# PaddlePaddle/PaddleFleetX

Measured on AMD Instinct MI355X. Metric: tokens/sec/GPU GPT-3-6.7B pretrain, DP2×TP2×PP2 at 1/2/4/8 MI355X, higher is better.
Workload: dtype bf16; 1 GPU; model=GPT-6.7B, global_batch=32, seq_len=1024, micro_batch=16, parallelism=dp1tp1pp1

## Files before the change

### csrc/attention.hip

```cpp
#include "common.h"

#include <torch/extension.h>
#include <ATen/hip/HIPContext.h>

namespace {

typedef __attribute__((ext_vector_type(8))) __bf16 bf8;
typedef __attribute__((ext_vector_type(4))) float f4;
typedef __attribute__((ext_vector_type(8))) short short8v;

#define MFMA_BF16(a, b, c) __builtin_amdgcn_mfma_f32_16x16x32_bf16(a, b, c, 0, 0, 0)

constexpr int TILE = 64;
constexpr int NWAVES = 4;
constexpr int BLOCKT = NWAVES * WAVE;
constexpr int PAD = 8;

constexpr int FW_WAVES = 8;
constexpr int FW_BLOCKT = FW_WAVES * WAVE;
constexpr int QTILE = FW_WAVES * 16;

struct Strided {
  const __hip_bfloat16* p;
  long bs, hs, rs;
  DEV_INLINE const __hip_bfloat16* at(int b, int h) const {
    return p + (long)b * bs + (long)h * hs;
  }
};
struct StridedMut {
  __hip_bfloat16* p;
  long bs, hs, rs;
  DEV_INLINE __hip_bfloat16* at(int b, int h) const {
    return p + (long)b * bs + (long)h * hs;
  }
};

template <int D>
DEV_INLINE void stage_rowmajor(const __hip_bfloat16* __restrict__ g, long rs,
                               int nvalid, unsigned short* lds) {
  constexpr int RS = D + PAD;
  constexpr int NV = TILE * D / 8;
  for (int v = threadIdx.x; v < NV; v += BLOCKT) {
    int row = v / (D / 8);
    int col = (v % (D / 8)) * 8;
    short4v lo = {0, 0, 0, 0}, hi = {0, 0, 0, 0};
    if (row < nvalid) {
      const unsigned short* src = (const unsigned short*)g + (long)row * rs + col;
      lo = *reinterpret_cast<const short4v*>(src);
      hi = *reinterpret_cast<const short4v*>(src + 4);
    }
    *reinterpret_cast<short4v*>(lds + row * RS + col) = lo;
    *reinterpret_cast<short4v*>(lds + row * RS + col + 4) = hi;
  }
}

template <int D>
DEV_INLINE void stage_both(const __hip_bfloat16* __restrict__ g, long rs,
                           int nvalid, unsigned short* lds_rm,
                           unsigned short* lds_tr) {
  constexpr int RSM = D + PAD;
  constexpr int RST = TILE + PAD;
  constexpr int NV = TILE * D / 8;
  for (int v = threadIdx.x; v < NV; v += BLOCKT) {
    int row = v / (D / 8);
    int col = (v % (D / 8)) * 8;
    short4v lo = {0, 0, 0, 0}, hi = {0, 0, 0, 0};
    if (row < nvalid) {
      const unsigned short* src = (const unsigned short*)g + (long)row * rs + col;
      lo = *reinterpret_cast<const short4v*>(src);
      hi = *reinterpret_cast<const short4v*>(src + 4);
    }
    *reinterpret_cast<short4v*>(lds_rm + row * RSM + col) = lo;
    *reinterpret_cast<short4v*>(lds_rm + row * RSM + col + 4) = hi;
    unsigned short tmp[8];
    *reinterpret_cast<short4v*>(tmp) = lo;
    *reinterpret_cast<short4v*>(tmp + 4) = hi;
#pragma unroll
    for (int j = 0; j < 8; ++j) lds_tr[(col + j) * RST + row] = tmp[j];
  }
}

template <int D>
DEV_INLINE void load_a_frags(const __hip_bfloat16* __restrict__ g, long rs,
                             int row0, int nvalid, int lane, bf8* frags) {
  int row = row0 + (lane & 15);
  int d0 = (lane >> 4) * 8;
#pragma unroll
  for (int kc = 0; kc < D / 32; ++kc) {
    bf8 f = {};
    if (row < nvalid) {
      const unsigned short* src =
          (const unsigned short*)g + (long)row * rs + kc * 32 + d0;
      union { short4v v[2]; bf8 b; } u;
      u.v[0] = *reinterpret_cast<const short4v*>(src);
      u.v[1] = *reinterpret_cast<const short4v*>(src + 4);
      f = u.b;
    }
    frags[kc] = f;
  }
}

DEV_INLINE bf8 read_b_frag(const unsigned short* lds, int row_stride, int col0,
                           int k0, int lane) {
  const unsigned short* p =
      lds + (col0 + (lane & 15)) * row_stride + k0 + (lane >> 4) * 8;
  union { short4v v[2]; bf8 b; } u;
  u.v[0] = *reinterpret_cast<const short4v*>(p);
  u.v[1] = *reinterpret_cast<const short4v*>(p + 4);
  return u.b;
}

DEV_INLINE bf8 read_a_frag_lds(const unsigned short* lds, int row_stride,
                               int k0, int lane) {
  const unsigned short* p =
      lds + (lane & 15) * row_stride + k0 + (lane >> 4) * 8;
  union { short4v v[2]; bf8 b; } u;
  u.v[0] = *reinterpret_cast<const short4v*>(p);
  u.v[1] = *reinterpret_cast<const short4v*>(p + 4);
  return u.b;
}

template <int D, bool CAUSAL, bool DROP>
__global__ __launch_bounds__(FW_BLOCKT) void attn_fwd_kernel(
    Strided q, Strided k, Strided v, StridedMut o, float* __restrict__ lse_out,
    int H, int S, float scale, int kv_total, int n_home,
    unsigned drop_thresh, float drop_inv_keep, unsigned seed0,
    unsigned seed1) {
  constexpr int KRS = D + PAD;
  constexpr int VRS = TILE + 4;
  constexpr int NDT = D / 16;
  constexpr int KSZ = TILE * KRS;
  constexpr int VSZ = D * VRS;

  __shared__ unsigned short smem[2 * KSZ + 2 * VSZ];
  unsigned short* k_lds = smem;
  unsigned short* vt_lds = smem + 2 * KSZ;

  const int b = blockIdx.x / H, hh = blockIdx.x % H;
  const long bh = blockIdx.x;
  const int wid = threadIdx.x / WAVE;
  const int lane = threadIdx.x % WAVE;

  const __hip_bfloat16* qp = q.at(b, hh);
  const __hip_bfloat16* kp = k.at(b, hh);
  const __hip_bfloat16* vp = v.at(b, hh);

  auto run_qtile = [&](const int qt) {

  constexpr int RB = 2;
  const int qrow0 = qt * (QTILE * RB) + wid * (16 * RB);
  bf8 qfrag[RB][D / 32];
#pragma unroll
  for (int rb = 0; rb < RB; ++rb)
    load_a_frags<D>(qp, q.rs, qrow0 + rb * 16, S, lane, qfrag[rb]);

  f4 oacc[RB][NDT];
#pragma unroll
  for (int rb = 0; rb < RB; ++rb)
#pragma unroll
    for (int i = 0; i < NDT; ++i) oacc[rb][i] = f4{0.f, 0.f, 0.f, 0.f};
  float m_r[RB][1], l_r[RB][1];
#pragma unroll
  for (int rb = 0; rb < RB; ++rb) { m_r[rb][0] = -INFINITY; l_r[rb][0] = 0.f; }

  const int ccol = lane & 15;
  const int crow4 = (lane >> 4) * 4;

  const int kv_tiles = CAUSAL
      ? min(kv_total, (qt * QTILE * RB + QTILE * RB - 1) / TILE + 1)
      : kv_total;

  constexpr int TPR = D / 16;
  const int st_row = threadIdx.x / TPR;
  const int st_col = (threadIdx.x % TPR) * 16;
  const bool st_on = st_row < TILE;
  constexpr int VCB = D / 4;
  const int vb_row = (threadIdx.x / VCB) * 4;
  const int vb_col = (threadIdx.x % VCB) * 4;
  const bool vb_on = vb_row < TILE;
  short8v kreg[2];
  short4v vblk[4];

  auto load_kv = [&](int kv0) {
#pragma unroll
    for (int h2 = 0; h2 < 2; ++h2) kreg[h2] = short8v{};
#pragma unroll
    for (int r = 0; r < 4; ++r) vblk[r] = short4v{};
    const int krow = kv0 + st_row;
    if (st_on && krow < S) {
      const unsigned short* ks = (const unsigned short*)kp +
                                 (long)krow * k.rs + st_col;
      kreg[0] = *reinterpret_cast<const short8v*>(ks);
      kreg[1] = *reinterpret_cast<const short8v*>(ks + 8);
    }
    if (vb_on) {
#pragma unroll
      for (int r = 0; r < 4; ++r) {
        const int vrow = kv0 + vb_row + r;
// ... 181 lines not shown
          oacc[rb][dt] = MFMA_BF16(pa[rb][kc], vb, oacc[rb][dt]);
      }
    }

    if (have_next)
      write_kv(k_lds + (cur ^ 1) * KSZ, vt_lds + (cur ^ 1) * VSZ);
    __syncthreads();
  }

  __hip_bfloat16* op = o.at(b, hh);
#pragma unroll
  for (int rb = 0; rb < RB; ++rb) {
    float inv_own = (l_r[rb][0] > 0.f) ? 1.f / l_r[rb][0] : 0.f;
    float inv4[4];
#pragma unroll
    for (int r = 0; r < 4; ++r) inv4[r] = __shfl(inv_own, crow4 + r, WAVE);
    if ((lane >> 4) == 0 && lse_out) {
      int qrow = qrow0 + rb * 16 + ccol;
      if (qrow < S)
        lse_out[bh * (long)S + qrow] =
            (l_r[rb][0] > 0.f) ? m_r[rb][0] + logf(l_r[rb][0]) : -INFINITY;
    }
#pragma unroll
    for (int r = 0; r < 4; ++r) {
      int qrow = qrow0 + rb * 16 + crow4 + r;
      if (qrow >= S) continue;
      unsigned short* orow = (unsigned short*)op + (long)qrow * o.rs;
#pragma unroll
      for (int dt = 0; dt < NDT; dt += 2) {
        unsigned int u = cvt_pk_bf16(oacc[rb][dt][r] * inv4[r],
                                     oacc[rb][dt + 1][r] * inv4[r]);
        orow[dt * 16 + ccol] = (unsigned short)u;
        orow[(dt + 1) * 16 + ccol] = (unsigned short)(u >> 16);
      }
    }
  }
  };

  const int n_home_abs = n_home < 0 ? -n_home : n_home;
  run_qtile(blockIdx.y);
  if (n_home < 0) {
    const int qt2 = (n_home_abs - 1) - (int)blockIdx.y;
    if (qt2 != (int)blockIdx.y && qt2 >= 0) {
      __syncthreads();
      run_qtile(qt2);
    }
  }
}

__global__ void attn_bwd_delta_kernel(Strided dout, Strided o,
                                      float* __restrict__ delta, long rows,
                                      int H, int S, int D) {
  constexpr int GROUPS = BLOCKT / 16;
  long row = (long)blockIdx.x * GROUPS + threadIdx.x / 16;
  if (row >= rows) return;
  int s = (int)(row % S);
  long bh = row / S;
  int hh = (int)(bh % H);
  int b = (int)(bh / H);
  int lane16 = threadIdx.x % 16;
  const unsigned short* dp =
      (const unsigned short*)dout.at(b, hh) + (long)s * dout.rs;
  const unsigned short* op = (const unsigned short*)o.at(b, hh) + (long)s * o.rs;
  float acc = 0.f;
  for (int i = lane16 * 4; i < D; i += 16 * 4) {
    short4v dv = *reinterpret_cast<const short4v*>(dp + i);
    short4v ov = *reinterpret_cast<const short4v*>(op + i);
#pragma unroll
    for (int j = 0; j < 4; ++j)
      acc += bf_raw2f(((unsigned short*)&dv)[j]) *
             bf_raw2f(((unsigned short*)&ov)[j]);
  }
  acc = group16_reduce_sum(acc);
  if (lane16 == 0) delta[bh * (long)S + s] = acc;
}

template <int D, bool CAUSAL, bool DROP>
__global__ __launch_bounds__(FW_BLOCKT) void attn_bwd_dkv_kernel(
    Strided q, Strided k, Strided v, Strided dout,
    const float* __restrict__ lse, const float* __restrict__ delta,
    StridedMut dk, StridedMut dv, int H, int S, float scale, int q_tiles,
    int n_home, unsigned drop_thresh, float drop_inv_keep, unsigned seed0,
    unsigned seed1) {
  constexpr int RS = D + PAD;
  constexpr int TS = TILE + PAD;
  constexpr int TRS = TILE + 4;
  constexpr int NDT = D / 16;
  constexpr int QSZ = TILE * RS;
  constexpr int TSZ = D * TRS;

  __shared__ unsigned short q_lds[2 * QSZ];
  __shared__ unsigned short qt_lds[2 * TSZ];
  __shared__ unsigned short do_lds[2 * QSZ];
  __shared__ unsigned short dot_lds[2 * TSZ];
  __shared__ unsigned short p_lds[FW_WAVES * 16 * TS];
  __shared__ float lsed_lds[2][2 * TILE];

  const int b = blockIdx.x / H, hh = blockIdx.x % H;
  const long bh = blockIdx.x;
  const int wid = threadIdx.x / WAVE;
  const int lane = threadIdx.x % WAVE;

  const __hip_bfloat16* qp = q.at(b, hh);
  const __hip_bfloat16* kp = k.at(b, hh);
  const __hip_bfloat16* vp = v.at(b, hh);
  const __hip_bfloat16* dop = dout.at(b, hh);

  auto run_kvtile = [&](const int kt) {
  const int kvrow0 = kt * QTILE + wid * 16;
  bf8 kfrag[D / 32], vfrag[D / 32];
  load_a_frags<D>(kp, k.rs, kvrow0, S, lane, kfrag);
  load_a_frags<D>(vp, v.rs, kvrow0, S, lane, vfrag);

  f4 dvacc[NDT], dkacc[NDT];
#pragma unroll
  for (int i = 0; i < NDT; ++i) {
    dvacc[i] = f4{0.f, 0.f, 0.f, 0.f};
    dkacc[i] = f4{0.f, 0.f, 0.f, 0.f};
  }

  const int ccol = lane & 15;
  const int crow4 = (lane >> 4) * 4;
  const int my_kvrow = kvrow0 + crow4;
  unsigned short* myp = p_lds + wid * 16 * TS;

  constexpr int TPR = D / 16;
  const int st_row = threadIdx.x / TPR;
  const int st_col = (threadIdx.x % TPR) * 16;
  const bool st_on = st_row < TILE;
  constexpr int VCB = D / 4;
  const int vb_row = (threadIdx.x / VCB) * 4;
  const int vb_col = (threadIdx.x % VCB) * 4;
  const bool vb_on = vb_row < TILE;
  short8v qreg[2], dreg[2];
  short4v qblk[4], dblk[4];
  float lse_s = 0.f, dlt_s = 0.f;

  const int qt_first = CAUSAL ? (kt * QTILE) / TILE : 0;

  auto issue_loads = [&](int q0) {
#pragma unroll
    for (int h2 = 0; h2 < 2; ++h2) { qreg[h2] = short8v{}; dreg[h2] = short8v{}; }
#pragma unroll
    for (int r = 0; r < 4; ++r) { qblk[r] = short4v{}; dblk[r] = short4v{}; }
    const int row = q0 + st_row;
    if (st_on && row < S) {
      const unsigned short* qs = (const unsigned short*)qp + (long)row * q.rs + st_col;
      const unsigned short* ds = (const unsigned short*)dop + (long)row * dout.rs + st_col;
      qreg[0] = *reinterpret_cast<const short8v*>(qs);
      qreg[1] = *reinterpret_cast<const short8v*>(qs + 8);
      dreg[0] = *reinterpret_cast<const short8v*>(ds);
      dreg[1] = *reinterpret_cast<const short8v*>(ds + 8);
    }
    if (vb_on) {
#pragma unroll
      for (int r = 0; r < 4; ++r) {
        const int vrow = q0 + vb_row + r;
        if (vrow < S) {
          qblk[r] = *reinterpret_cast<const short4v*>(
              (const unsigned short*)qp + (long)vrow * q.rs + vb_col);
          dblk[r] = *reinterpret_cast<const short4v*>(
              (const unsigned short*)dop + (long)vrow * dout.rs + vb_col);
        }
      }
    }
    const int li = threadIdx.x;
    if (li < TILE) {
      int qi = q0 + li;
      lse_s = (qi < S) ? lse[bh * (long)S + qi] : 0.f;
      dlt_s = (qi < S) ? delta[bh * (long)S + qi] : 0.f;
    }
  };
  auto write_tiles = [&](int buf) {
    unsigned short* qd = q_lds + buf * QSZ;
    unsigned short* dd = do_lds + buf * QSZ;
    unsigned short* qtd = qt_lds + buf * TSZ;
    unsigned short* dtd = dot_lds + buf * TSZ;
    if (st_on) {
      *reinterpret_cast<short8v*>(qd + st_row * RS + st_col) = qreg[0];
      *reinterpret_cast<short8v*>(qd + st_row * RS + st_col + 8) = qreg[1];
      *reinterpret_cast<short8v*>(dd + st_row * RS + st_col) = dreg[0];
      *reinterpret_cast<short8v*>(dd + st_row * RS + st_col + 8) = dreg[1];
    }
    if (vb_on) {
#pragma unroll
      for (int c = 0; c < 4; ++c) {
        short4v tq = {qblk[0][c], qblk[1][c], qblk[2][c], qblk[3][c]};
        short4v td = {dblk[0][c], dblk[1][c], dblk[2][c], dblk[3][c]};
        *reinterpret_cast<short4v*>(qtd + (vb_col + c) * TRS + vb_row) = tq;
        *reinterpret_cast<short4v*>(dtd + (vb_col + c) * TRS + vb_row) = td;
      }
    }
    if (threadIdx.x < TILE) {
      lsed_lds[buf][threadIdx.x] = lse_s;
      lsed_lds[buf][TILE + threadIdx.x] = dlt_s;
    }
  };

  issue_loads(qt_first * TILE);
  write_tiles(0);
  __syncthreads();

  for (int qt = qt_first; qt < q_tiles; ++qt) {
    const int q0 = qt * TILE;
    const int cur = (qt - qt_first) & 1;
    const unsigned short* qb_lds = q_lds + cur * QSZ;
    const unsigned short* db_lds = do_lds + cur * QSZ;
    const unsigned short* qtb_lds = qt_lds + cur * TSZ;
    const unsigned short* dtb_lds = dot_lds + cur * TSZ;
    const float* lsed_b = lsed_lds[cur];
    const bool have_next = (qt + 1) < q_tiles;
    if (have_next) issue_loads(q0 + TILE);

    const bool active = !CAUSAL || (q0 + TILE - 1 >= kvrow0);
    f4 pt[4], dpt[4];
    if (active) {
      unsigned dmask[4];
#pragma unroll
      for (int ct = 0; ct < 4; ++ct) {
        f4 acc = {0.f, 0.f, 0.f, 0.f};
#pragma unroll
        for (int kc = 0; kc < D / 32; ++kc) {
          bf8 qb = read_b_frag(qb_lds, RS, ct * 16, kc * 32, lane);
          acc = MFMA_BF16(kfrag[kc], qb, acc);
        }
        int qcol = q0 + ct * 16 + ccol;
        float l = lsed_b[ct * 16 + ccol];
#pragma unroll
        for (int r = 0; r < 4; ++r) {
          int kvr = my_kvrow + r;
          float p = 0.f;
          if ((!CAUSAL || qcol >= kvr) && qcol < S && kvr < S)
            p = __expf(acc[r] * scale - l);
          pt[ct][r] = p;
        }
        if constexpr (DROP) {
          philox4 r4 = philox4x32_10((unsigned)qcol,
                                     (unsigned)(my_kvrow >> 2),
                                     (unsigned)bh, seed1, seed0, seed1);
          const unsigned rr[4] = {r4.x, r4.y, r4.z, r4.w};
          unsigned m = 0;
#pragma unroll
          for (int r = 0; r < 4; ++r)
            if (rr[r] >= drop_thresh) m |= (1u << r);
          dmask[ct] = m;
        }
      }

#pragma unroll
      for (int ct = 0; ct < 4; ++ct)
#pragma unroll
        for (int r = 0; r < 4; r += 2) {
          float p0 = pt[ct][r], p1 = pt[ct][r + 1];
          if constexpr (DROP) {
            p0 = (dmask[ct] >> r) & 1 ? p0 * drop_inv_keep : 0.f;
            p1 = (dmask[ct] >> (r + 1)) & 1 ? p1 * drop_inv_keep : 0.f;
          }
          unsigned int u = cvt_pk_bf16(p0, p1);
          unsigned short* base = myp + (crow4 + r) * TS + ct * 16 + ccol;
          base[0] = (unsigned short)u;
          base[TS] = (unsigned short)(u >> 16);
        }
#pragma unroll
      for (int kc = 0; kc < 2; ++kc) {
        bf8 pa = read_a_frag_lds(myp, TS, kc * 32, lane);
#pragma unroll
        for (int dt = 0; dt < NDT; ++dt) {
          bf8 db = read_b_frag(dtb_lds, TRS, dt * 16, kc * 32, lane);
          dvacc[dt] = MFMA_BF16(pa, db, dvacc[dt]);
        }
      }

#pragma unroll
      for (int ct = 0; ct < 4; ++ct) {
        f4 acc = {0.f, 0.f, 0.f, 0.f};
#pragma unroll
        for (int kc = 0; kc < D / 32; ++kc) {
          bf8 db = read_b_frag(db_lds, RS, ct * 16, kc * 32, lane);
          acc = MFMA_BF16(vfrag[kc], db, acc);
        }
        dpt[ct] = acc;
      }

#pragma unroll
      for (int ct = 0; ct < 4; ++ct) {
        float dlt = lsed_b[TILE + ct * 16 + ccol];
        float ds[4];
#pragma unroll
        for (int r = 0; r < 4; ++r) {
          float dp = dpt[ct][r];
          if constexpr (DROP)
            dp = (dmask[ct] >> r) & 1 ? dp * drop_inv_keep : 0.f;
          ds[r] = pt[ct][r] * (dp - dlt) * scale;
        }
#pragma unroll
        for (int r = 0; r < 4; r += 2) {
          unsigned int u = cvt_pk_bf16(ds[r], ds[r + 1]);
          unsigned short* base = myp + (crow4 + r) * TS + ct * 16 + ccol;
          base[0] = (unsigned short)u;
          base[TS] = (unsigned short)(u >> 16);
        }
      }
#pragma unroll
      for (int kc = 0; kc < 2; ++kc) {
        bf8 dsa = read_a_frag_lds(myp, TS, kc * 32, lane);
#pragma unroll
        for (int dt = 0; dt < NDT; ++dt) {
          bf8 qb = read_b_frag(qtb_lds, TRS, dt * 16, kc * 32, lane);
          dkacc[dt] = MFMA_BF16(dsa, qb, dkacc[dt]);
        }
      }
    }

    if (have_next) write_tiles(cur ^ 1);
    __syncthreads();
  }

  __hip_bfloat16* dkp = dk.at(b, hh);
  __hip_bfloat16* dvp = dv.at(b, hh);
#pragma unroll
  for (int r = 0; r < 4; ++r) {
    int kvr = my_kvrow + r;
    if (kvr >= S) continue;
    unsigned short* krow = (unsigned short*)dkp + (long)kvr * dk.rs;
    unsigned short* vrow = (unsigned short*)dvp + (long)kvr * dv.rs;
#pragma unroll
    for (int dt = 0; dt < NDT; dt += 2) {
      unsigned int uk = cvt_pk_bf16(dkacc[dt][r], dkacc[dt + 1][r]);
      unsigned int uv = cvt_pk_bf16(dvacc[dt][r], dvacc[dt + 1][r]);
      krow[dt * 16 + ccol] = (unsigned short)uk;
      krow[(dt + 1) * 16 + ccol] = (unsigned short)(uk >> 16);
      vrow[dt * 16 + ccol] = (unsigned short)uv;
      vrow[(dt + 1) * 16 + ccol] = (unsigned short)(uv >> 16);
    }
  }
  };

  const int n_home_abs = n_home < 0 ? -n_home : n_home;
  run_kvtile(blockIdx.y);
  if (n_home < 0) {
    const int kt2 = (n_home_abs - 1) - (int)blockIdx.y;
    if (kt2 != (int)blockIdx.y && kt2 >= 0) {
      __syncthreads();
      run_kvtile(kt2);
    }
  }
}

template <int D, bool CAUSAL, bool DROP>
__global__ __launch_bounds__(FW_BLOCKT) void attn_bwd_dq_kernel(
    Strided q, Strided k, Strided v, Strided dout,
    const float* __restrict__ lse, const float* __restrict__ delta,
    StridedMut dq, int H, int S, float scale, int kv_total, int n_home,
    unsigned drop_thresh, float drop_inv_keep, unsigned seed0,
    unsigned seed1) {
  constexpr int RS = D + PAD;
  constexpr int TS = TILE + PAD;
  constexpr int TRS = TILE + 4;
  constexpr int NDT = D / 16;
  constexpr int KSZ = TILE * RS;
  constexpr int TSZ = D * TRS;
  constexpr int VSZ = TILE * RS;
  constexpr int RB = 2;

  __shared__ unsigned short smem[2 * (KSZ + TSZ + VSZ) + FW_WAVES * 32 * TS];
  unsigned short* k_lds = smem;
  unsigned short* kt_lds = smem + 2 * KSZ;
  unsigned short* v_lds = smem + 2 * (KSZ + TSZ);
  unsigned short* p_lds = smem + 2 * (KSZ + TSZ + VSZ);

  const int b = blockIdx.x / H, hh = blockIdx.x % H;
  const long bh = blockIdx.x;
  const int wid = threadIdx.x / WAVE;
  const int lane = threadIdx.x % WAVE;

  const __hip_bfloat16* qp = q.at(b, hh);
  const __hip_bfloat16* kp = k.at(b, hh);
  const __hip_bfloat16* vp = v.at(b, hh);
  const __hip_bfloat16* dop = dout.at(b, hh);

  auto run_qtile = [&](const int qt) {
  const int qrow0 = qt * (QTILE * RB) + wid * (16 * RB);
  bf8 qfrag[RB][D / 32], dofrag[RB][D / 32];
#pragma unroll
  for (int rb = 0; rb < RB; ++rb) {
    load_a_frags<D>(qp, q.rs, qrow0 + rb * 16, S, lane, qfrag[rb]);
    load_a_frags<D>(dop, dout.rs, qrow0 + rb * 16, S, lane, dofrag[rb]);
  }

  f4 dqacc[RB][NDT];
#pragma unroll
  for (int rb = 0; rb < RB; ++rb)
#pragma unroll
    for (int i = 0; i < NDT; ++i) dqacc[rb][i] = f4{0.f, 0.f, 0.f, 0.f};

  const int ccol = lane & 15;
  const int crow4 = (lane >> 4) * 4;
  unsigned short* myp = p_lds + wid * 32 * TS;

  float lse_r[RB][4], dlt_r[RB][4];
#pragma unroll
  for (int rb = 0; rb < RB; ++rb)
#pragma unroll
    for (int r = 0; r < 4; ++r) {
      int qr = qrow0 + rb * 16 + crow4 + r;
      lse_r[rb][r] = (qr < S) ? lse[bh * (long)S + qr] : 0.f;
      dlt_r[rb][r] = (qr < S) ? delta[bh * (long)S + qr] : 0.f;
    }

  const int kv_tiles = CAUSAL
      ? min(kv_total, (qt * QTILE * RB + QTILE * RB - 1) / TILE + 1)
      : kv_total;
  const int wave_last_row = min(qrow0 + RB * 16 - 1, S - 1);

  constexpr int TPR = D / 16;
  const int st_row = threadIdx.x / TPR;
  const int st_col = (threadIdx.x % TPR) * 16;
  const bool st_on = st_row < TILE;
  constexpr int VCB = D / 4;
  const int vb_row = (threadIdx.x / VCB) * 4;
  const int vb_col = (threadIdx.x % VCB) * 4;
  const bool vb_on = vb_row < TILE;
  short8v kreg[2], vreg[2];
  short4v kblk[4];

  auto issue_loads = [&](int kv0) {
#pragma unroll
    for (int h2 = 0; h2 < 2; ++h2) { kreg[h2] = short8v{}; vreg[h2] = short8v{}; }
#pragma unroll
    for (int r = 0; r < 4; ++r) kblk[r] = short4v{};
    const int row = kv0 + st_row;
    if (st_on && row < S) {
      const unsigned short* ks = (const unsigned short*)kp + (long)row * k.rs + st_col;
      const unsigned short* vs = (const unsigned short*)vp + (long)row * v.rs + st_col;
      kreg[0] = *reinterpret_cast<const short8v*>(ks);
      kreg[1] = *reinterpret_cast<const short8v*>(ks + 8);
      vreg[0] = *reinterpret_cast<const short8v*>(vs);
      vreg[1] = *reinterpret_cast<const short8v*>(vs + 8);
    }
    if (vb_on) {
#pragma unroll
      for (int r = 0; r < 4; ++r) {
        const int vrow = kv0 + vb_row + r;
        if (vrow < S)
          kblk[r] = *reinterpret_cast<const short4v*>(
              (const unsigned short*)kp + (long)vrow * k.rs + vb_col);
      }
    }
  };
  auto write_tiles = [&](int buf) {
    unsigned short* kd = k_lds + buf * KSZ;
    unsigned short* ktd = kt_lds + buf * TSZ;
    unsigned short* vd = v_lds + buf * VSZ;
    if (st_on) {
      *reinterpret_cast<short8v*>(kd + st_row * RS + st_col) = kreg[0];
      *reinterpret_cast<short8v*>(kd + st_row * RS + st_col + 8) = kreg[1];
      *reinterpret_cast<short8v*>(vd + st_row * RS + st_col) = vreg[0];
      *reinterpret_cast<short8v*>(vd + st_row * RS + st_col + 8) = vreg[1];
    }
    if (vb_on) {
#pragma unroll
      for (int c = 0; c < 4; ++c) {
        short4v t = {kblk[0][c], kblk[1][c], kblk[2][c], kblk[3][c]};
        *reinterpret_cast<short4v*>(ktd + (vb_col + c) * TRS + vb_row) = t;
      }
    }
  };

  issue_loads(0);
  write_tiles(0);
  __syncthreads();

  for (int ktl = 0; ktl < kv_tiles; ++ktl) {
    const int kv0 = ktl * TILE;
    const int cur = ktl & 1;
    const unsigned short* kb_lds = k_lds + cur * KSZ;
    const unsigned short* ktb_lds = kt_lds + cur * TSZ;
    const unsigned short* vb_lds = v_lds + cur * VSZ;

    const bool have_next = (ktl + 1) < kv_tiles;
    if (have_next) issue_loads(kv0 + TILE);

    const bool active = !CAUSAL || (kv0 <= wave_last_row);
    if (active) {
#pragma unroll
      for (int ct = 0; ct < 4; ++ct) {
        f4 sacc[RB], dpacc[RB];
#pragma unroll
        for (int rb = 0; rb < RB; ++rb) {
          sacc[rb] = f4{0.f, 0.f, 0.f, 0.f};
          dpacc[rb] = f4{0.f, 0.f, 0.f, 0.f};
        }
#pragma unroll
        for (int kc = 0; kc < D / 32; ++kc) {
          bf8 kb = read_b_frag(kb_lds, RS, ct * 16, kc * 32, lane);
#pragma unroll
          for (int rb = 0; rb < RB; ++rb)
            sacc[rb] = MFMA_BF16(qfrag[rb][kc], kb, sacc[rb]);
        }
#pragma unroll
        for (int kc = 0; kc < D / 32; ++kc) {
          bf8 vb = read_b_frag(vb_lds, RS, ct * 16, kc * 32, lane);
#pragma unroll
          for (int rb = 0; rb < RB; ++rb)
            dpacc[rb] = MFMA_BF16(dofrag[rb][kc], vb, dpacc[rb]);
        }
        int kcol = kv0 + ct * 16 + ccol;
#pragma unroll
        for (int rb = 0; rb < RB; ++rb) {
          const int row_base = qrow0 + rb * 16 + crow4;
          float ds[4];
#pragma unroll
          for (int r = 0; r < 4; ++r) {
            float pv = 0.f;
            if ((!CAUSAL || kcol <= row_base + r) && kcol < S &&
                row_base + r < S)
              pv = __expf(sacc[rb][r] * scale - lse_r[rb][r]);
            float dp = dpacc[rb][r];
            if constexpr (DROP) {
              philox4 r4 = philox4x32_10((unsigned)(row_base + r),
                                         (unsigned)(kcol >> 2),
                                         (unsigned)bh, seed1, seed0, seed1);
              const unsigned rr[4] = {r4.x, r4.y, r4.z, r4.w};
              dp = (rr[kcol & 3] >= drop_thresh) ? dp * drop_inv_keep : 0.f;
            }
            ds[r] = pv * (dp - dlt_r[rb][r]) * scale;
          }
#pragma unroll
          for (int r = 0; r < 4; r += 2) {
            unsigned int u = cvt_pk_bf16(ds[r], ds[r + 1]);
            unsigned short* base =
                myp + (rb * 16 + crow4 + r) * TS + ct * 16 + ccol;
            base[0] = (unsigned short)u;
            base[TS] = (unsigned short)(u >> 16);
          }
        }
      }

      bf8 dsa[RB][2];
#pragma unroll
      for (int rb = 0; rb < RB; ++rb)
#pragma unroll
        for (int kc = 0; kc < 2; ++kc)
          dsa[rb][kc] = read_a_frag_lds(myp + rb * 16 * TS, TS, kc * 32,
                                        lane);
#pragma unroll
      for (int kc = 0; kc < 2; ++kc) {
#pragma unroll
        for (int dt = 0; dt < NDT; ++dt) {
          bf8 kb = read_b_frag(ktb_lds, TRS, dt * 16, kc * 32, lane);
#pragma unroll
          for (int rb = 0; rb < RB; ++rb)
            dqacc[rb][dt] = MFMA_BF16(dsa[rb][kc], kb, dqacc[rb][dt]);
        }
      }
    }

    if (have_next) write_tiles(cur ^ 1);
    __syncthreads();
  }

  __hip_bfloat16* dqp = dq.at(b, hh);
#pragma unroll
  for (int rb = 0; rb < RB; ++rb)
#pragma unroll
    for (int r = 0; r < 4; ++r) {
      int qr = qrow0 + rb * 16 + crow4 + r;
      if (qr >= S) continue;
      unsigned short* qrow_p = (unsigned short*)dqp + (long)qr * dq.rs;
#pragma unroll
      for (int dt = 0; dt < NDT; dt += 2) {
        unsigned int u = cvt_pk_bf16(dqacc[rb][dt][r],
                                     dqacc[rb][dt + 1][r]);
        qrow_p[dt * 16 + ccol] = (unsigned short)u;
        qrow_p[(dt + 1) * 16 + ccol] = (unsigned short)(u >> 16);
      }
    }
  };

  const int n_home_abs = n_home < 0 ? -n_home : n_home;
  run_qtile(blockIdx.y);
  if (n_home < 0) {
    const int qt2 = (n_home_abs - 1) - (int)blockIdx.y;
    if (qt2 != (int)blockIdx.y && qt2 >= 0) {
      __syncthreads();
      run_qtile(qt2);
    }
  }
}

Strided strided_of(const torch::Tensor& t, int b_dim, int h_dim, int s_dim) {
  Strided s;
  s.p = (const __hip_bfloat16*)t.data_ptr();
  s.bs = t.stride(b_dim);
  s.hs = t.stride(h_dim);
  s.rs = t.stride(s_dim);
  return s;
}
StridedMut strided_mut_of(torch::Tensor& t, int b_dim, int h_dim, int s_dim) {
  StridedMut s;
  s.p = (__hip_bfloat16*)t.data_ptr();
  s.bs = t.stride(b_dim);
  s.hs = t.stride(h_dim);
  s.rs = t.stride(s_dim);
  return s;
}

void check_attn_tensor(const torch::Tensor& t, int d_dim, int D) {
  TORCH_CHECK(t.is_cuda() && t.scalar_type() == torch::kBFloat16);
  TORCH_CHECK(t.size(d_dim) == D && t.stride(d_dim) == 1,
              "head_dim axis must be contiguous");
}

void launch_fwd(Strided q, Strided k, Strided v, StridedMut o, float* lse,
                int B, int H, int S, int D, float scale, bool causal,
                float p_drop = 0.f, unsigned long long seed = 0) {
  int q_blocks = (S + QTILE * 2 - 1) / (QTILE * 2);
  int kv_total = (S + TILE - 1) / TILE;
  bool pair = causal && B * H < 256 && q_blocks > 1;
  int grid_y = pair ? (q_blocks + 1) / 2 : q_blocks;
  int n_home = pair ? -q_blocks : q_blocks;
  dim3 grid(B * H, grid_y);
  auto stream = at::hip::getCurrentHIPStream();
  unsigned thresh = (unsigned)(p_drop * 4294967296.0);
  float invk = 1.f / (1.f - p_drop);
  unsigned s0 = (unsigned)seed, s1 = (unsigned)(seed >> 32);
  bool drop = p_drop > 0.f;
#define LAUNCH_FWD(DD, CC, PP)                                              \
  hipLaunchKernelGGL((attn_fwd_kernel<DD, CC, PP>), grid, dim3(FW_BLOCKT),  \
                     0, stream, q, k, v, o, lse, H, S, scale, kv_total,     \
                     n_home, thresh, invk, s0, s1)
#define PICK_FWD(DD, CC) do { if (drop) LAUNCH_FWD(DD, CC, true); \
                              else LAUNCH_FWD(DD, CC, false); } while (0)
  if (D == 128) { if (causal) PICK_FWD(128, true); else PICK_FWD(128, false); }
  else          { if (causal) PICK_FWD(64, true);  else PICK_FWD(64, false); }
#undef PICK_FWD
#undef LAUNCH_FWD
}

void launch_bwd(Strided q, Strided k, Strided v, Strided dout, Strided o,
                StridedMut dq, StridedMut dk, StridedMut dv, float* lse,
                float* delta, int B, int H, int S, int D, float scale,
                bool causal, float p_drop = 0.f,
                unsigned long long seed = 0) {
  auto stream = at::hip::getCurrentHIPStream();
  long rows = (long)B * H * S;
  hipLaunchKernelGGL(attn_bwd_delta_kernel,
                     dim3((rows + (BLOCKT / 16) - 1) / (BLOCKT / 16)),
                     dim3(BLOCKT), 0, stream, dout, o, delta, rows, H, S, D);
  int tiles64 = (S + TILE - 1) / TILE;
  int blocks128 = (S + QTILE - 1) / QTILE;
  int blocks256 = (S + QTILE * 2 - 1) / (QTILE * 2);
  bool pair = causal && B * H < 256;
  int nh_dkv = (pair && blocks128 > 1) ? -blocks128 : blocks128;
  int nh_dq = (pair && blocks256 > 1) ? -blocks256 : blocks256;
  dim3 grid(B * H, nh_dkv < 0 ? (blocks128 + 1) / 2 : blocks128);
  dim3 grid_dq(B * H, nh_dq < 0 ? (blocks256 + 1) / 2 : blocks256);
  unsigned thresh = (unsigned)(p_drop * 4294967296.0);
  float invk = 1.f / (1.f - p_drop);
  unsigned s0 = (unsigned)seed, s1 = (unsigned)(seed >> 32);
  bool drop = p_drop > 0.f;
#define LAUNCH_BWD(DD, CC, PP)                                               \
  do {                                                                       \
    hipLaunchKernelGGL((attn_bwd_dkv_kernel<DD, CC, PP>), grid,              \
                       dim3(FW_BLOCKT), 0, stream, q, k, v, dout, lse,       \
                       delta, dk, dv, H, S, scale, tiles64, nh_dkv, thresh,  \
                       invk, s0, s1);                                        \
    hipLaunchKernelGGL((attn_bwd_dq_kernel<DD, CC, PP>), grid_dq,            \
                       dim3(FW_BLOCKT), 0, stream, q, k, v, dout, lse,       \
                       delta, dq, H, S, scale, tiles64, nh_dq, thresh,       \
                       invk, s0, s1);                                        \
  } while (0)
// ... 97 lines not shown
```

Baseline: 26210 tokens/s.

## Use transposed LDS reads and register-resident P/dS in attention backward

Rewrites the dK/dV and dQ backward kernels so score and dP tiles are computed in transposed orientation. P and dS then stay in registers as packed MFMA operands instead of round-tripping through per-wave LDS scratch. The separately staged transposed copies of Q, dO and K are replaced by ds_read_tr16_b64 transposed reads from a single row-permuted LDS image, and outputs are written as packed 4-element stores. This cuts LDS footprint and staging traffic, but relies on a nontrivial row permutation and lane mapping that must be exactly right for correctness.

```diff
diff --git a/csrc/attention.hip b/csrc/attention.hip
--- a/csrc/attention.hip
+++ b/csrc/attention.hip
@@ -35,49 +35,44 @@
   }
 };
 
-template <int D>
-DEV_INLINE void stage_rowmajor(const __hip_bfloat16* __restrict__ g, long rs,
-                               int nvalid, unsigned short* lds) {
-  constexpr int RS = D + PAD;
-  constexpr int NV = TILE * D / 8;
-  for (int v = threadIdx.x; v < NV; v += BLOCKT) {
-    int row = v / (D / 8);
-    int col = (v % (D / 8)) * 8;
-    short4v lo = {0, 0, 0, 0}, hi = {0, 0, 0, 0};
-    if (row < nvalid) {
-      const unsigned short* src = (const unsigned short*)g + (long)row * rs + col;
-      lo = *reinterpret_cast<const short4v*>(src);
-      hi = *reinterpret_cast<const short4v*>(src + 4);
-    }
-    *reinterpret_cast<short4v*>(lds + row * RS + col) = lo;
-    *reinterpret_cast<short4v*>(lds + row * RS + col + 4) = hi;
-  }
-}
-
-template <int D>
-DEV_INLINE void stage_both(const __hip_bfloat16* __restrict__ g, long rs,
-                           int nvalid, unsigned short* lds_rm,
-                           unsigned short* lds_tr) {
-  constexpr int RSM = D + PAD;
-  constexpr int RST = TILE + PAD;
-  constexpr int NV = TILE * D / 8;
-  for (int v = threadIdx.x; v < NV; v += BLOCKT) {
-    int row = v / (D / 8);
-    int col = (v % (D / 8)) * 8;
-    short4v lo = {0, 0, 0, 0}, hi = {0, 0, 0, 0};
-    if (row < nvalid) {
-      const unsigned short* src = (const unsigned short*)g + (long)row * rs + col;
-      lo = *reinterpret_cast<const short4v*>(src);
-      hi = *reinterpret_cast<const short4v*>(src + 4);
-    }
-    *reinterpret_cast<short4v*>(lds_rm + row * RSM + col) = lo;
-    *reinterpret_cast<short4v*>(lds_rm + row * RSM + col + 4) = hi;
-    unsigned short tmp[8];
-    *reinterpret_cast<short4v*>(tmp) = lo;
-    *reinterpret_cast<short4v*>(tmp + 4) = hi;
-#pragma unroll
-    for (int j = 0; j < 8; ++j) lds_tr[(col + j) * RST + row] = tmp[j];
-  }
+constexpr int BPAD = 16;
+
+DEV_INLINE int img_row(int R) {
+  return (R & 0x23) | ((R & 0x18) >> 1) | ((R & 0x4) << 2);
+}
+
+typedef __attribute__((address_space(3))) short4v lds_short4v;
+
+DEV_INLINE bf8 read_rows_frag(const unsigned short* lds, int row_stride,
+                              int k0, int lane) {
+  const unsigned short* p =
+      lds + (lane & 15) * row_stride + k0 + (lane >> 4) * 8;
+  union { short8v v; bf8 b; } u;
+  u.v = *reinterpret_cast<const short8v*>(p);
+  return u.b;
+}
+
+DEV_INLINE int tr_lane_offset(int row_stride, int lane) {
+  return ((lane >> 4) * 4 + ((lane & 15) >> 2)) * row_stride + (lane & 3) * 4;
+}
+
+DEV_INLINE bf8 read_tr_frag(const unsigned short* img_lane, int row_stride,
+                            int r0, int c0) {
+  const unsigned short* p = img_lane + r0 * row_stride + c0;
+  union { short4v v[2]; bf8 b; } u;
+  u.v[0] = __builtin_amdgcn_ds_read_tr16_b64_v4i16((lds_short4v*)p);
+  u.v[1] = __builtin_amdgcn_ds_read_tr16_b64_v4i16(
+      (lds_short4v*)(p + 16 * row_stride));
+  return u.b;
+}
+
+DEV_INLINE bf8 pack_acc_frag(const f4& lo, const f4& hi) {
+  union { unsigned int u[4]; bf8 b; } r;
+  r.u[0] = cvt_pk_bf16(lo[0], lo[1]);
+  r.u[1] = cvt_pk_bf16(lo[2], lo[3]);
+  r.u[2] = cvt_pk_bf16(hi[0], hi[1]);
+  r.u[3] = cvt_pk_bf16(hi[2], hi[3]);
+  return r.b;
 }
 
 template <int D>
@@ -104,16 +99,6 @@
                            int k0, int lane) {
   const unsigned short* p =
       lds + (col0 + (lane & 15)) * row_stride + k0 + (lane >> 4) * 8;
-  union { short4v v[2]; bf8 b; } u;
-  u.v[0] = *reinterpret_cast<const short4v*>(p);
-  u.v[1] = *reinterpret_cast<const short4v*>(p + 4);
-  return u.b;
-}
-
-DEV_INLINE bf8 read_a_frag_lds(const unsigned short* lds, int row_stride,
-                               int k0, int lane) {
-  const unsigned short* p =
-      lds + (lane & 15) * row_stride + k0 + (lane >> 4) * 8;
   union { short4v v[2]; bf8 b; } u;
   u.v[0] = *reinterpret_cast<const short4v*>(p);
   u.v[1] = *reinterpret_cast<const short4v*>(p + 4);
@@ -461,23 +446,17 @@
     StridedMut dk, StridedMut dv, int H, int S, float scale, int q_tiles,
     int n_home, unsigned drop_thresh, float drop_inv_keep, unsigned seed0,
     unsigned seed1) {
-  constexpr int RS = D + PAD;
-  constexpr int TS = TILE + PAD;
-  constexpr int TRS = TILE + 4;
+  constexpr int RS = D + BPAD;
   constexpr int NDT = D / 16;
   constexpr int QSZ = TILE * RS;
-  constexpr int TSZ = D * TRS;
-
-  __shared__ unsigned short q_lds[2 * QSZ];
-  __shared__ unsigned short qt_lds[2 * TSZ];
-  __shared__ unsigned short do_lds[2 * QSZ];
-  __shared__ unsigned short dot_lds[2 * TSZ];
-  __shared__ unsigned short p_lds[FW_WAVES * 16 * TS];
-  __shared__ float lsed_lds[2][2 * TILE];
+
+  __shared__ __attribute__((aligned(16))) unsigned short q_lds[2 * QSZ];
+  __shared__ __attribute__((aligned(16))) unsigned short do_lds[2 * QSZ];
+  __shared__ __attribute__((aligned(16))) float lsed_lds[2][2 * TILE];
 
   const int b = blockIdx.x / H, hh = blockIdx.x % H;
   const long bh = blockIdx.x;
-  const int wid = threadIdx.x / WAVE;
+  const int wid = __builtin_amdgcn_readfirstlane(threadIdx.x / WAVE);
   const int lane = threadIdx.x % WAVE;
 
   const __hip_bfloat16* qp = q.at(b, hh);
@@ -500,19 +479,14 @@
 
   const int ccol = lane & 15;
   const int crow4 = (lane >> 4) * 4;
-  const int my_kvrow = kvrow0 + crow4;
-  unsigned short* myp = p_lds + wid * 16 * TS;
+  const int my_kv = kvrow0 + ccol;
+  const int tr_off = tr_lane_offset(RS, lane);
 
   constexpr int TPR = D / 16;
   const int st_row = threadIdx.x / TPR;
   const int st_col = (threadIdx.x % TPR) * 16;
   const bool st_on = st_row < TILE;
-  constexpr int VCB = D / 4;
-  const int vb_row = (threadIdx.x / VCB) * 4;
-  const int vb_col = (threadIdx.x % VCB) * 4;
-  const bool vb_on = vb_row < TILE;
   short8v qreg[2], dreg[2];
-  short4v qblk[4], dblk[4];
   float lse_s = 0.f, dlt_s = 0.f;
 
   const int qt_first = CAUSAL ? (kt * QTILE) / TILE : 0;
@@ -520,8 +494,6 @@
   auto issue_loads = [&](int q0) {
 #pragma unroll
     for (int h2 = 0; h2 < 2; ++h2) { qreg[h2] = short8v{}; dreg[h2] = short8v{}; }
-#pragma unroll
-    for (int r = 0; r < 4; ++r) { qblk[r] = short4v{}; dblk[r] = short4v{}; }
     const int row = q0 + st_row;
     if (st_on && row < S) {
       const unsigned short* qs = (const unsigned short*)qp + (long)row * q.rs + st_col;
@@ -531,18 +503,6 @@
       dreg[0] = *reinterpret_cast<const short8v*>(ds);
       dreg[1] = *reinterpret_cast<const short8v*>(ds + 8);
     }
-    if (vb_on) {
-#pragma unroll
-      for (int r = 0; r < 4; ++r) {
-        const int vrow = q0 + vb_row + r;
-        if (vrow < S) {
-          qblk[r] = *reinterpret_cast<const short4v*>(
-              (const unsigned short*)qp + (long)vrow * q.rs + vb_col);
-          dblk[r] = *reinterpret_cast<const short4v*>(
-              (const unsigned short*)dop + (long)vrow * dout.rs + vb_col);
-        }
-      }
-    }
     const int li = threadIdx.x;
     if (li < TILE) {
       int qi = q0 + li;
@@ -553,22 +513,12 @@
   auto write_tiles = [&](int buf) {
     unsigned short* qd = q_lds + buf * QSZ;
     unsigned short* dd = do_lds + buf * QSZ;
-    unsigned short* qtd = qt_lds + buf * TSZ;
-    unsigned short* dtd = dot_lds + buf * TSZ;
     if (st_on) {
-      *reinterpret_cast<short8v*>(qd + st_row * RS + st_col) = qreg[0];
-      *reinterpret_cast<short8v*>(qd + st_row * RS + st_col + 8) = qreg[1];
-      *reinterpret_cast<short8v*>(dd + st_row * RS + st_col) = dreg[0];
-      *reinterpret_cast<short8v*>(dd + st_row * RS + st_col + 8) = dreg[1];
-    }
-    if (vb_on) {
-#pragma unroll
-      for (int c = 0; c < 4; ++c) {
-        short4v tq = {qblk[0][c], qblk[1][c], qblk[2][c], qblk[3][c]};
-        short4v td = {dblk[0][c], dblk[1][c], dblk[2][c], dblk[3][c]};
-        *reinterpret_cast<short4v*>(qtd + (vb_col + c) * TRS + vb_row) = tq;
-        *reinterpret_cast<short4v*>(dtd + (vb_col + c) * TRS + vb_row) = td;
-      }
+      const int ir = img_row(st_row);
+      *reinterpret_cast<short8v*>(qd + ir * RS + st_col) = qreg[0];
+      *reinterpret_cast<short8v*>(qd + ir * RS + st_col + 8) = qreg[1];
+      *reinterpret_cast<short8v*>(dd + ir * RS + st_col) = dreg[0];
+      *reinterpret_cast<short8v*>(dd + ir * RS + st_col + 8) = dreg[1];
     }
     if (threadIdx.x < TILE) {
       lsed_lds[buf][threadIdx.x] = lse_s;
@@ -585,108 +535,58 @@
     const int cur = (qt - qt_first) & 1;
     const unsigned short* qb_lds = q_lds + cur * QSZ;
     const unsigned short* db_lds = do_lds + cur * QSZ;
-    const unsigned short* qtb_lds = qt_lds + cur * TSZ;
-    const unsigned short* dtb_lds = dot_lds + cur * TSZ;
     const float* lsed_b = lsed_lds[cur];
     const bool have_next = (qt + 1) < q_tiles;
     if (have_next) issue_loads(q0 + TILE);
 
     const bool active = !CAUSAL || (q0 + TILE - 1 >= kvrow0);
-    f4 pt[4], dpt[4];
     if (active) {
-      unsigned dmask[4];
-#pragma unroll
-      for (int ct = 0; ct < 4; ++ct) {
-        f4 acc = {0.f, 0.f, 0.f, 0.f};
-#pragma unroll
-        for (int kc = 0; kc < D / 32; ++kc) {
-          bf8 qb = read_b_frag(qb_lds, RS, ct * 16, kc * 32, lane);
-          acc = MFMA_BF16(kfrag[kc], qb, acc);
-        }
-        int qcol = q0 + ct * 16 + ccol;
-        float l = lsed_b[ct * 16 + ccol];
-#pragma unroll
-        for (int r = 0; r < 4; ++r) {
-          int kvr = my_kvrow + r;
-          float p = 0.f;
-          if ((!CAUSAL || qcol >= kvr) && qcol < S && kvr < S)
-            p = __expf(acc[r] * scale - l);
-          pt[ct][r] = p;
-        }
-        if constexpr (DROP) {
-          philox4 r4 = philox4x32_10((unsigned)qcol,
-                                     (unsigned)(my_kvrow >> 2),
-                                     (unsigned)bh, seed1, seed0, seed1);
-          const unsigned rr[4] = {r4.x, r4.y, r4.z, r4.w};
-          unsigned m = 0;
-#pragma unroll
-          for (int r = 0; r < 4; ++r)
-            if (rr[r] >= drop_thresh) m |= (1u << r);
-          dmask[ct] = m;
-        }
-      }
-
-#pragma unroll
-      for (int ct = 0; ct < 4; ++ct)
-#pragma unroll
-        for (int r = 0; r < 4; r += 2) {
-          float p0 = pt[ct][r], p1 = pt[ct][r + 1];
-          if constexpr (DROP) {
-            p0 = (dmask[ct] >> r) & 1 ? p0 * drop_inv_keep : 0.f;
-            p1 = (dmask[ct] >> (r + 1)) & 1 ? p1 * drop_inv_keep : 0.f;
+#pragma unroll
+      for (int j = 0; j < 2; ++j) {
+        f4 pd[2], ds[2];
+#pragma unroll
+        for (int h = 0; h < 2; ++h) {
+          const int t = 2 * j + h;
+          f4 sacc = {0.f, 0.f, 0.f, 0.f}, dpacc = {0.f, 0.f, 0.f, 0.f};
+#pragma unroll
+          for (int kc = 0; kc < D / 32; ++kc) {
+            bf8 qa = read_rows_frag(qb_lds + t * 16 * RS, RS, kc * 32, lane);
+            bf8 da = read_rows_frag(db_lds + t * 16 * RS, RS, kc * 32, lane);
+            sacc = MFMA_BF16(qa, kfrag[kc], sacc);
+            dpacc = MFMA_BF16(da, vfrag[kc], dpacc);
           }
-          unsigned int u = cvt_pk_bf16(p0, p1);
-          unsigned short* base = myp + (crow4 + r) * TS + ct * 16 + ccol;
-          base[0] = (unsigned short)u;
-          base[TS] = (unsigned short)(u >> 16);
-        }
-#pragma unroll
-      for (int kc = 0; kc < 2; ++kc) {
-        bf8 pa = read_a_frag_lds(myp, TS, kc * 32, lane);
+          const int tr4 = 32 * j + 2 * crow4 + 4 * h;
+          const f4 l4 = *reinterpret_cast<const f4*>(lsed_b + tr4);
+          const f4 d4 = *reinterpret_cast<const f4*>(lsed_b + TILE + tr4);
+#pragma unroll
+          for (int r = 0; r < 4; ++r) {
+            const int qrow = q0 + tr4 + r;
+            const float e = __expf(sacc[r] * scale - l4[r]);
+            const bool valid =
+                (!CAUSAL || qrow >= my_kv) && qrow < S && my_kv < S;
+            const float p = valid ? e : 0.f;
+            float pdv = p, dp = dpacc[r];
+            if constexpr (DROP) {
+              philox4 r4 = philox4x32_10((unsigned)qrow,
+                                         (unsigned)(my_kv >> 2),
+                                         (unsigned)bh, seed1, seed0, seed1);
+              const unsigned rr[4] = {r4.x, r4.y, r4.z, r4.w};
+              const bool keep = rr[my_kv & 3] >= drop_thresh;
+              pdv = keep ? p * drop_inv_keep : 0.f;
+              dp = keep ? dp * drop_inv_keep : 0.f;
+            }
+            pd[h][r] = pdv;
+            ds[h][r] = p * (dp - d4[r]) * scale;
+          }
+        }
+        const bf8 pfrag = pack_acc_frag(pd[0], pd[1]);
+        const bf8 dsfrag = pack_acc_frag(ds[0], ds[1]);
 #pragma unroll
         for (int dt = 0; dt < NDT; ++dt) {
-          bf8 db = read_b_frag(dtb_lds, TRS, dt * 16, kc * 32, lane);
-          dvacc[dt] = MFMA_BF16(pa, db, dvacc[dt]);
-        }
-      }
-
-#pragma unroll
-      for (int ct = 0; ct < 4; ++ct) {
-        f4 acc = {0.f, 0.f, 0.f, 0.f};
-#pragma unroll
-        for (int kc = 0; kc < D / 32; ++kc) {
-          bf8 db = read_b_frag(db_lds, RS, ct * 16, kc * 32, lane);
-          acc = MFMA_BF16(vfrag[kc], db, acc);
-        }
-        dpt[ct] = acc;
-      }
-
-#pragma unroll
-      for (int ct = 0; ct < 4; ++ct) {
-        float dlt = lsed_b[TILE + ct * 16 + ccol];
-        float ds[4];
-#pragma unroll
-        for (int r = 0; r < 4; ++r) {
-          float dp = dpt[ct][r];
-          if constexpr (DROP)
-            dp = (dmask[ct] >> r) & 1 ? dp * drop_inv_keep : 0.f;
-          ds[r] = pt[ct][r] * (dp - dlt) * scale;
-        }
-#pragma unroll
-        for (int r = 0; r < 4; r += 2) {
-          unsigned int u = cvt_pk_bf16(ds[r], ds[r + 1]);
-          unsigned short* base = myp + (crow4 + r) * TS + ct * 16 + ccol;
-          base[0] = (unsigned short)u;
-          base[TS] = (unsigned short)(u >> 16);
-        }
-      }
-#pragma unroll
-      for (int kc = 0; kc < 2; ++kc) {
-        bf8 dsa = read_a_frag_lds(myp, TS, kc * 32, lane);
-#pragma unroll
-        for (int dt = 0; dt < NDT; ++dt) {
-          bf8 qb = read_b_frag(qtb_lds, TRS, dt * 16, kc * 32, lane);
-          dkacc[dt] = MFMA_BF16(dsa, qb, dkacc[dt]);
+          bf8 dta = read_tr_frag(db_lds + tr_off, RS, 32 * j, dt * 16);
+          dvacc[dt] = MFMA_BF16(dta, pfrag, dvacc[dt]);
+          bf8 qta = read_tr_frag(qb_lds + tr_off, RS, 32 * j, dt * 16);
+          dkacc[dt] = MFMA_BF16(qta, dsfrag, dkacc[dt]);
         }
       }
     }
@@ -695,22 +595,20 @@
     __syncthreads();
   }
 
-  __hip_bfloat16* dkp = dk.at(b, hh);
-  __hip_bfloat16* dvp = dv.at(b, hh);
-#pragma unroll
-  for (int r = 0; r < 4; ++r) {
-    int kvr = my_kvrow + r;
-    if (kvr >= S) continue;
-    unsigned short* krow = (unsigned short*)dkp + (long)kvr * dk.rs;
-    unsigned short* vrow = (unsigned short*)dvp + (long)kvr * dv.rs;
-#pragma unroll
-    for (int dt = 0; dt < NDT; dt += 2) {
-      unsigned int uk = cvt_pk_bf16(dkacc[dt][r], dkacc[dt + 1][r]);
-      unsigned int uv = cvt_pk_bf16(dvacc[dt][r], dvacc[dt + 1][r]);
-      krow[dt * 16 + ccol] = (unsigned short)uk;
-      krow[(dt + 1) * 16 + ccol] = (unsigned short)(uk >> 16);
-      vrow[dt * 16 + ccol] = (unsigned short)uv;
-      vrow[(dt + 1) * 16 + ccol] = (unsigned short)(uv >> 16);
+  if (my_kv < S) {
+    unsigned short* krow =
+        (unsigned short*)dk.at(b, hh) + (long)my_kv * dk.rs + crow4;
+    unsigned short* vrow =
+        (unsigned short*)dv.at(b, hh) + (long)my_kv * dv.rs + crow4;
+#pragma unroll
+    for (int dt = 0; dt < NDT; ++dt) {
+      union { unsigned int u[2]; short4v v; } pk, pv;
+      pk.u[0] = cvt_pk_bf16(dkacc[dt][0], dkacc[dt][1]);
+      pk.u[1] = cvt_pk_bf16(dkacc[dt][2], dkacc[dt][3]);
+      pv.u[0] = cvt_pk_bf16(dvacc[dt][0], dvacc[dt][1]);
+      pv.u[1] = cvt_pk_bf16(dvacc[dt][2], dvacc[dt][3]);
+      *reinterpret_cast<short4v*>(krow + dt * 16) = pk.v;
+      *reinterpret_cast<short4v*>(vrow + dt * 16) = pv.v;
     }
   }
   };
@@ -733,24 +631,17 @@
     StridedMut dq, int H, int S, float scale, int kv_total, int n_home,
     unsigned drop_thresh, float drop_inv_keep, unsigned seed0,
     unsigned seed1) {
-  constexpr int RS = D + PAD;
-  constexpr int TS = TILE + PAD;
-  constexpr int TRS = TILE + 4;
+  constexpr int RS = D + BPAD;
   constexpr int NDT = D / 16;
   constexpr int KSZ = TILE * RS;
-  constexpr int TSZ = D * TRS;
-  constexpr int VSZ = TILE * RS;
   constexpr int RB = 2;
 
-  __shared__ unsigned short smem[2 * (KSZ + TSZ + VSZ) + FW_WAVES * 32 * TS];
-  unsigned short* k_lds = smem;
-  unsigned short* kt_lds = smem + 2 * KSZ;
-  unsigned short* v_lds = smem + 2 * (KSZ + TSZ);
-  unsigned short* p_lds = smem + 2 * (KSZ + TSZ + VSZ);
+  __shared__ __attribute__((aligned(16))) unsigned short k_lds[2 * KSZ];
+  __shared__ __attribute__((aligned(16))) unsigned short v_lds[2 * KSZ];
 
   const int b = blockIdx.x / H, hh = blockIdx.x % H;
   const long bh = blockIdx.x;
-  const int wid = threadIdx.x / WAVE;
+  const int wid = __builtin_amdgcn_readfirstlane(threadIdx.x / WAVE);
   const int lane = threadIdx.x % WAVE;
 
   const __hip_bfloat16* qp = q.at(b, hh);
@@ -775,17 +666,16 @@
 
   const int ccol = lane & 15;
   const int crow4 = (lane >> 4) * 4;
-  unsigned short* myp = p_lds + wid * 32 * TS;
-
-  float lse_r[RB][4], dlt_r[RB][4];
-#pragma unroll
-  for (int rb = 0; rb < RB; ++rb)
-#pragma unroll
-    for (int r = 0; r < 4; ++r) {
-      int qr = qrow0 + rb * 16 + crow4 + r;
-      lse_r[rb][r] = (qr < S) ? lse[bh * (long)S + qr] : 0.f;
-      dlt_r[rb][r] = (qr < S) ? delta[bh * (long)S + qr] : 0.f;
-    }
+  const int tr_off = tr_lane_offset(RS, lane);
+
+  int my_q[RB];
+  float lse_r[RB], dlt_r[RB];
+#pragma unroll
+  for (int rb = 0; rb < RB; ++rb) {
+    my_q[rb] = qrow0 + rb * 16 + ccol;
+    lse_r[rb] = (my_q[rb] < S) ? lse[bh * (long)S + my_q[rb]] : 0.f;
+    dlt_r[rb] = (my_q[rb] < S) ? delta[bh * (long)S + my_q[rb]] : 0.f;
+  }
 
   const int kv_tiles = CAUSAL
       ? min(kv_total, (qt * QTILE * RB + QTILE * RB - 1) / TILE + 1)
@@ -796,18 +686,11 @@
   const int st_row = threadIdx.x / TPR;
   const int st_col = (threadIdx.x % TPR) * 16;
   const bool st_on = st_row < TILE;
-  constexpr int VCB = D / 4;
-  const int vb_row = (threadIdx.x / VCB) * 4;
-  const int vb_col = (threadIdx.x % VCB) * 4;
-  const bool vb_on = vb_row < TILE;
   short8v kreg[2], vreg[2];
-  short4v kblk[4];
 
   auto issue_loads = [&](int kv0) {
 #pragma unroll
     for (int h2 = 0; h2 < 2; ++h2) { kreg[h2] = short8v{}; vreg[h2] = short8v{}; }
-#pragma unroll
-    for (int r = 0; r < 4; ++r) kblk[r] = short4v{};
     const int row = kv0 + st_row;
     if (st_on && row < S) {
       const unsigned short* ks = (const unsigned short*)kp + (long)row * k.rs + st_col;
@@ -817,32 +700,16 @@
       vreg[0] = *reinterpret_cast<const short8v*>(vs);
       vreg[1] = *reinterpret_cast<const short8v*>(vs + 8);
     }
-    if (vb_on) {
-#pragma unroll
-      for (int r = 0; r < 4; ++r) {
-        const int vrow = kv0 + vb_row + r;
-        if (vrow < S)
-          kblk[r] = *reinterpret_cast<const short4v*>(
-              (const unsigned short*)kp + (long)vrow * k.rs + vb_col);
-      }
-    }
   };
   auto write_tiles = [&](int buf) {
     unsigned short* kd = k_lds + buf * KSZ;
-    unsigned short* ktd = kt_lds + buf * TSZ;
-    unsigned short* vd = v_lds + buf * VSZ;
+    unsigned short* vd = v_lds + buf * KSZ;
     if (st_on) {
-      *reinterpret_cast<short8v*>(kd + st_row * RS + st_col) = kreg[0];
-      *reinterpret_cast<short8v*>(kd + st_row * RS + st_col + 8) = kreg[1];
-      *reinterpret_cast<short8v*>(vd + st_row * RS + st_col) = vreg[0];
-      *reinterpret_cast<short8v*>(vd + st_row * RS + st_col + 8) = vreg[1];
-    }
-    if (vb_on) {
-#pragma unroll
-      for (int c = 0; c < 4; ++c) {
-        short4v t = {kblk[0][c], kblk[1][c], kblk[2][c], kblk[3][c]};
-        *reinterpret_cast<short4v*>(ktd + (vb_col + c) * TRS + vb_row) = t;
-      }
+      const int ir = img_row(st_row);
+      *reinterpret_cast<short8v*>(kd + ir * RS + st_col) = kreg[0];
+      *reinterpret_cast<short8v*>(kd + ir * RS + st_col + 8) = kreg[1];
+      *reinterpret_cast<short8v*>(vd + ir * RS + st_col) = vreg[0];
+      *reinterpret_cast<short8v*>(vd + ir * RS + st_col + 8) = vreg[1];
     }
   };
 
@@ -854,8 +721,7 @@
     const int kv0 = ktl * TILE;
     const int cur = ktl & 1;
     const unsigned short* kb_lds = k_lds + cur * KSZ;
-    const unsigned short* ktb_lds = kt_lds + cur * TSZ;
-    const unsigned short* vb_lds = v_lds + cur * VSZ;
+    const unsigned short* vb_lds = v_lds + cur * KSZ;
 
     const bool have_next = (ktl + 1) < kv_tiles;
     if (have_next) issue_loads(kv0 + TILE);
@@ -863,74 +729,62 @@
     const bool active = !CAUSAL || (kv0 <= wave_last_row);
     if (active) {
 #pragma unroll
-      for (int ct = 0; ct < 4; ++ct) {
-        f4 sacc[RB], dpacc[RB];
-#pragma unroll
-        for (int rb = 0; rb < RB; ++rb) {
-          sacc[rb] = f4{0.f, 0.f, 0.f, 0.f};
-          dpacc[rb] = f4{0.f, 0.f, 0.f, 0.f};
-        }
-#pragma unroll
-        for (int kc = 0; kc < D / 32; ++kc) {
-          bf8 kb = read_b_frag(kb_lds, RS, ct * 16, kc * 32, lane);
+      for (int j = 0; j < 2; ++j) {
+        f4 ds[RB][2];
+#pragma unroll
+        for (int h = 0; h < 2; ++h) {
+          const int t = 2 * j + h;
+          f4 sacc[RB], dpacc[RB];
+#pragma unroll
+          for (int rb = 0; rb < RB; ++rb) {
+            sacc[rb] = f4{0.f, 0.f, 0.f, 0.f};
+            dpacc[rb] = f4{0.f, 0.f, 0.f, 0.f};
+          }
+#pragma unroll
+          for (int kc = 0; kc < D / 32; ++kc) {
+            bf8 ka = read_rows_frag(kb_lds + t * 16 * RS, RS, kc * 32, lane);
+            bf8 va = read_rows_frag(vb_lds + t * 16 * RS, RS, kc * 32, lane);
+#pragma unroll
+            for (int rb = 0; rb < RB; ++rb)
+              sacc[rb] = MFMA_BF16(ka, qfrag[rb][kc], sacc[rb]);
+#pragma unroll
+            for (int rb = 0; rb < RB; ++rb)
+              dpacc[rb] = MFMA_BF16(va, dofrag[rb][kc], dpacc[rb]);
+          }
+          const int kv4 = kv0 + 32 * j + 2 * crow4 + 4 * h;
+#pragma unroll
+          for (int rb = 0; rb < RB; ++rb) {
+            unsigned rr[4] = {0u, 0u, 0u, 0u};
+            if constexpr (DROP) {
+              philox4 r4 = philox4x32_10((unsigned)my_q[rb],
+                                         (unsigned)(kv4 >> 2), (unsigned)bh,
+                                         seed1, seed0, seed1);
+              rr[0] = r4.x; rr[1] = r4.y; rr[2] = r4.z; rr[3] = r4.w;
+            }
+#pragma unroll
+            for (int r = 0; r < 4; ++r) {
+              const int kvr = kv4 + r;
+              const float e = __expf(sacc[rb][r] * scale - lse_r[rb]);
+              const bool valid =
+                  (!CAUSAL || kvr <= my_q[rb]) && kvr < S && my_q[rb] < S;
+              const float pv = valid ? e : 0.f;
+              float dp = dpacc[rb][r];
+              if constexpr (DROP)
+                dp = (rr[r] >= drop_thresh) ? dp * drop_inv_keep : 0.f;
+              ds[rb][h][r] = pv * (dp - dlt_r[rb]) * scale;
+            }
+          }
+        }
+        bf8 dsfrag[RB];
+#pragma unroll
+        for (int rb = 0; rb < RB; ++rb)
+          dsfrag[rb] = pack_acc_frag(ds[rb][0], ds[rb][1]);
+#pragma unroll
+        for (int dt = 0; dt < NDT; ++dt) {
+          bf8 kta = read_tr_frag(kb_lds + tr_off, RS, 32 * j, dt * 16);
 #pragma unroll
           for (int rb = 0; rb < RB; ++rb)
-            sacc[rb] = MFMA_BF16(qfrag[rb][kc], kb, sacc[rb]);
-        }
-#pragma unroll
-        for (int kc = 0; kc < D / 32; ++kc) {
-          bf8 vb = read_b_frag(vb_lds, RS, ct * 16, kc * 32, lane);
-#pragma unroll
-          for (int rb = 0; rb < RB; ++rb)
-            dpacc[rb] = MFMA_BF16(dofrag[rb][kc], vb, dpacc[rb]);
-        }
-        int kcol = kv0 + ct * 16 + ccol;
-#pragma unroll
-        for (int rb = 0; rb < RB; ++rb) {
-          const int row_base = qrow0 + rb * 16 + crow4;
-          float ds[4];
-#pragma unroll
-          for (int r = 0; r < 4; ++r) {
-            float pv = 0.f;
-            if ((!CAUSAL || kcol <= row_base + r) && kcol < S &&
-                row_base + r < S)
-              pv = __expf(sacc[rb][r] * scale - lse_r[rb][r]);
-            float dp = dpacc[rb][r];
-            if constexpr (DROP) {
-              philox4 r4 = philox4x32_10((unsigned)(row_base + r),
-                                         (unsigned)(kcol >> 2),
-                                         (unsigned)bh, seed1, seed0, seed1);
-              const unsigned rr[4] = {r4.x, r4.y, r4.z, r4.w};
-              dp = (rr[kcol & 3] >= drop_thresh) ? dp * drop_inv_keep : 0.f;
-            }
-            ds[r] = pv * (dp - dlt_r[rb][r]) * scale;
-          }
-#pragma unroll
-          for (int r = 0; r < 4; r += 2) {
-            unsigned int u = cvt_pk_bf16(ds[r], ds[r + 1]);
-            unsigned short* base =
-                myp + (rb * 16 + crow4 + r) * TS + ct * 16 + ccol;
-            base[0] = (unsigned short)u;
-            base[TS] = (unsigned short)(u >> 16);
-          }
-        }
-      }
-
-      bf8 dsa[RB][2];
-#pragma unroll
-      for (int rb = 0; rb < RB; ++rb)
-#pragma unroll
-        for (int kc = 0; kc < 2; ++kc)
-          dsa[rb][kc] = read_a_frag_lds(myp + rb * 16 * TS, TS, kc * 32,
-                                        lane);
-#pragma unroll
-      for (int kc = 0; kc < 2; ++kc) {
-#pragma unroll
-        for (int dt = 0; dt < NDT; ++dt) {
-          bf8 kb = read_b_frag(ktb_lds, TRS, dt * 16, kc * 32, lane);
-#pragma unroll
-          for (int rb = 0; rb < RB; ++rb)
-            dqacc[rb][dt] = MFMA_BF16(dsa[rb][kc], kb, dqacc[rb][dt]);
+            dqacc[rb][dt] = MFMA_BF16(kta, dsfrag[rb], dqacc[rb][dt]);
         }
       }
     }
@@ -939,22 +793,19 @@
     __syncthreads();
   }
 
-  __hip_bfloat16* dqp = dq.at(b, hh);
-#pragma unroll
-  for (int rb = 0; rb < RB; ++rb)
-#pragma unroll
-    for (int r = 0; r < 4; ++r) {
-      int qr = qrow0 + rb * 16 + crow4 + r;
-      if (qr >= S) continue;
-      unsigned short* qrow_p = (unsigned short*)dqp + (long)qr * dq.rs;
-#pragma unroll
-      for (int dt = 0; dt < NDT; dt += 2) {
-        unsigned int u = cvt_pk_bf16(dqacc[rb][dt][r],
-                                     dqacc[rb][dt + 1][r]);
-        qrow_p[dt * 16 + ccol] = (unsigned short)u;
-        qrow_p[(dt + 1) * 16 + ccol] = (unsigned short)(u >> 16);
-      }
-    }
+#pragma unroll
+  for (int rb = 0; rb < RB; ++rb) {
+    if (my_q[rb] >= S) continue;
+    unsigned short* qrow_p =
+        (unsigned short*)dq.at(b, hh) + (long)my_q[rb] * dq.rs + crow4;
+#pragma unroll
+    for (int dt = 0; dt < NDT; ++dt) {
+      union { unsigned int u[2]; short4v v; } pk;
+      pk.u[0] = cvt_pk_bf16(dqacc[rb][dt][0], dqacc[rb][dt][1]);
+      pk.u[1] = cvt_pk_bf16(dqacc[rb][dt][2], dqacc[rb][dt][3]);
+      *reinterpret_cast<short4v*>(qrow_p + dt * 16) = pk.v;
+    }
+  }
   };
 
   const int n_home_abs = n_home < 0 ? -n_home : n_home;
@@ -967,6 +818,7 @@
     }
   }
 }
+
 
 Strided strided_of(const torch::Tensor& t, int b_dim, int h_dim, int s_dim) {
   Strided s;
```

New measurement: 26610 tokens/s, median of 3. About the same (+1.5%).
